# roymor1/OptimalStrategiesAgainstGenerativeAttacks

Measured on AMD Instinct MI355X. Metric: GIM episodes/sec (64x64x3, m=1 n=5 k=10), higher is better.
Workload: dtype f32

## Files before the change

### include/gim_hip.h

```cpp
#ifndef GIM_HIP_H
#define GIM_HIP_H

#include <stddef.h>
#include <stdint.h>

#ifdef __cplusplus
extern "C" {
#endif

#define GIM_OK 0
#define GIM_E_BADARG (-1)
#define GIM_E_LAUNCH (-2)

const char* gim_last_error(void);
int gim_version(void);

typedef struct {
    int32_t N, H, W, Cin, Cout, KH, ups;
    float pre_slope;
    int32_t pool, wfold, res_ups;
    int32_t tune_tile, tune_ksplit, tune_wgrad;
    int32_t out_zeroed;
    float post_slope;
    int32_t prec;
} gim_conv_shape;

int gim_conv2d_fold_weights(const float* w, float* f, int Cout, int Cin, int KH, void* stream);
typedef struct {
    const float* w;
    float* f;
    int32_t Cout, Cin, KH, reserved;
} gim_fold_job;
int gim_conv2d_fold_weights_batched(const gim_fold_job* jobs, const int32_t* tab, int n_blocks, void* stream);

int gim_conv2d_fwd(const float* x, const float* w, const float* bias, const float* sigma, const float* residual,
// ... 24 lines not shown
    int32_t Cout, Cin, KH, reserved;
} gim_sn_job;
int gim_spectral_sigma_batched(const gim_sn_job* jobs, int n_jobs, const int32_t* tab_cols, int n_col_blocks,
                               const int32_t* tab_rows, int n_row_blocks, float* out_base, int training, void* stream);

int gim_conv2d_transpose_weights(const float* w, float* wt, int Cout, int Cin, int KF, void* stream);
int gim_conv2d_dgrad_t(const float* dy, const float* wt, const float* sigma, const float* mask_x, float* dx,
                       const gim_conv_shape* shape, void* stream);

int gim_conv2d_xfold_weights(const float* w, float* wx, int Cout, int Cin, int KH, int J, void* stream);
int gim_conv2d_dgrad_xfold(const float* dy, const float* wx, const float* sigma, const float* mask_x, float* dx,
                           const gim_conv_shape* shape, int J, void* stream);

int gim_pad_image(const float* x, float* xp, int N, int H, int W, int C, int pad, float slope, void* stream);
int gim_conv2d_pack_rows_weights(const float* w, float* wp, int Cout, int Cin, int KH, void* stream);
int gim_conv2d_fwd_rows(const float* xp, const float* wp, const float* bias, const float* sigma, const float* residual,
                        float* y, const gim_conv_shape* shape, void* stream);
int gim_conv2d_wgrad_rows_acc(const float* dy, const float* xp, float* acc, float* bias_acc, const gim_conv_shape* shape, void* stream);

int gim_conv2d_pack_subpixel_weights(const float* wf, float* wm, int Cout, int Cin, int KH, void* stream);
int gim_depth_to_space2(const float* y4, const float* bias, float* y, int N, int Hs, int Ws, int C, float post_slope, void* stream);

int gim_conv_launch_plan(const gim_conv_shape* shape, int kind, int32_t* out);

int gim_conv2d_wgrad_acc(const float* dy, const float* x, float* acc, float* bias_acc, const gim_conv_shape* shape, void* stream);

typedef struct {
    const float* src;
    const float* bias_src;
    const float* w;
    const float* sigma;
    const float* u;
    const float* v;
    float* tmp;
    float* partial;
    float* grad_w;
    float* grad_b;
    int32_t Cout, Cin, K, fold;
    int32_t n_chunks, exclusive;
} gim_wgrad_job;
int gim_wgrad_finish_batched(const gim_wgrad_job* jobs, int n_jobs, const int32_t* tab, int n_blocks, const int32_t* tab_sn,
                             int n_blocks_sn, void* stream);

int gim_colsum(const float* x, float* out, float* scratch, int64_t rows, int C, void* stream);

int gim_colsum_acc(const float* x, float* out, float* scratch, int64_t rows, int C, void* stream);
// ... 154 lines not shown
```

### optimalstrategiesagainstgenerativeattacks_amd/_lib.py

```python
import ctypes
import os
from ctypes import POINTER, c_float, c_int, c_int32, c_int64, c_uint64, c_void_p

_HERE = os.path.dirname(os.path.abspath(__file__))
LIB_PATH = os.environ.get("GIM_LIB_PATH") or os.path.join(_HERE, "csrc", "libgim_hip.so")


class GimConvShape(ctypes.Structure):
    _fields_ = [("N", c_int32), ("H", c_int32), ("W", c_int32), ("Cin", c_int32), ("Cout", c_int32),
                ("KH", c_int32), ("ups", c_int32), ("pre_slope", c_float),
                ("pool", c_int32), ("wfold", c_int32), ("res_ups", c_int32),
                ("tune_tile", c_int32), ("tune_ksplit", c_int32), ("tune_wgrad", c_int32),
                ("out_zeroed", c_int32), ("post_slope", c_float), ("prec", c_int32)]


class GimInferConv(ctypes.Structure):
    _fields_ = [("N", c_int32), ("H", c_int32), ("W", c_int32), ("Cin", c_int32), ("Cout", c_int32),
                ("KH", c_int32), ("stride", c_int32)]


P = c_void_p
SP = POINTER(GimConvShape)


class GimFoldJob(ctypes.Structure):
    _fields_ = [("w", P), ("f", P), ("Cout", c_int32), ("Cin", c_int32), ("KH", c_int32), ("reserved", c_int32)]


class GimSnJob(ctypes.Structure):
    _fields_ = [("w", P), ("u", P), ("v", P), ("off_sigma", c_int64), ("off_u", c_int64), ("off_v", c_int64), ("off_scratch", c_int64),
                ("Cout", c_int32), ("Cin", c_int32), ("KH", c_int32), ("reserved", c_int32)]


class GimWgradJob(ctypes.Structure):
    _fields_ = [("src", P), ("bias_src", P), ("w", P), ("sigma", P), ("u", P), ("v", P), ("tmp", P), ("partial", P),
                ("grad_w", P), ("grad_b", P), ("Cout", c_int32), ("Cin", c_int32), ("K", c_int32), ("fold", c_int32),
# ... 35 lines not shown
    "gim_bgemm_grouped": [P, P, c_int, P],
    "gim_colsum_grouped": [P, P, c_int, P],
    "gim_scale_add_fwd": [P, P, P, P, c_int64, P],
    "gim_scale_add_fwd_act": [P, P, P, P, c_int64, c_float, P],
    "gim_scale_add_bwd": [P, P, P, P, P, P, c_int64, P],
    "gim_tanh_fwd": [P, P, c_int64, P],
    "gim_tanh_bwd": [P, P, P, c_int64, P],
    "gim_nchw_to_nhwc": [P, P, c_int, c_int, c_int, P],
    "gim_nhwc_to_nchw": [P, P, c_int, c_int, c_int, P],
    "gim_set_stats_fwd": [P, P, P, c_int, c_int, c_int, c_int64, c_int64, P],
    "gim_set_stats_bwd": [P, P, P, P, c_int, c_int, c_int, c_int64, c_int64, P],
    "gim_bce_logits_fwd": [P, P, c_float, c_int, P],
    "gim_bce_logits_bwd": [P, P, P, c_float, c_int, P],
    "gim_sum_dim1": [P, P, c_int, c_int, c_int, c_float, P],
    "gim_repeat_dim1": [P, P, c_int, c_int, c_int, c_float, P],
    "gim_noise_combine": [P, P, P, c_int, c_int, c_int, c_int, P],
    "gim_concat2": [P, P, P, c_int64, c_int, c_int, c_int, c_int, P],
    "gim_slice_channels": [P, P, c_int64, c_int, c_int, P],
    "gim_conv2d_wgrad_acc": [P, P, P, P, SP, P],
    "gim_wgrad_finish_batched": [P, c_int, P, c_int, P, c_int, P],
    "gim_colsum_acc": [P, P, P, c_int64, c_int, P],
    "gim_colsum2": [P, P, P, P, c_int, c_int, c_int, P],
    "gim_conv_launch_plan": [SP, c_int, P],
    "gim_conv2d_transpose_weights": [P, P, c_int, c_int, c_int, P],
    "gim_conv2d_dgrad_t": [P, P, P, P, P, SP, P],
    "gim_conv2d_xfold_weights": [P, P, c_int, c_int, c_int, c_int, P],
    "gim_conv2d_dgrad_xfold": [P, P, P, P, P, SP, c_int, P],
    "gim_episode_gather": [P, P, P, P, c_int, c_int, c_int, c_int, P],
    "gim_resize_bilinear_u8": [P, c_int64, c_int, c_int, c_int, c_int, P, c_int, c_int, P, P, c_int, P, P, c_int, P],
    "gim_maxpool_gather": [P, P, P, P, c_int, c_int, c_int, c_float, P],
    "gim_softmax_dim1_bwd_dp": [P, P, P, P, c_int, c_int, c_int, P],
    "gim_set_stats_bwd_bwd": [P, P, P, P, P, P, c_int, c_int, c_int, c_int64, c_int64, P],
    "gim_lrelu_mask_mul": [P, P, c_float, P, c_int64, P],
    "gim_sqsum_rows_fwd": [P, P, c_int, c_int64, P],
    "gim_sqsum_rows_bwd": [P, P, P, c_int, c_int64, P],
    "gim_img_att_mix_fwd": [P, P, P, P, P, P, P, P, c_int64, c_int, P],
    "gim_img_att_mix_bwd": [P, P, P, P, P, P, P, P, P, P, P, P, P, P, c_int64, c_int, P],
    "gim_adam_step": [P, P, P, P, c_int64, P, P, c_int, c_float, c_float, c_float, c_float, P, P],
    "gim_adam_step_scaled": [P, P, P, P, c_int64, P, P, c_int, c_float, c_float, c_float, c_float, P, P, P],
    "gim_spin": [c_int, P],
    "gim_pad_image": [P, P, c_int, c_int, c_int, c_int, c_int, c_float, P],
    "gim_conv2d_pack_rows_weights": [P, P, c_int, c_int, c_int, P],
    "gim_conv2d_pack_subpixel_weights": [P, P, c_int, c_int, c_int, P],
    "gim_depth_to_space2": [P, P, P, c_int, c_int, c_int, c_int, c_float, P],
    "gim_conv2d_fwd_rows": [P, P, P, P, P, P, SP, P],
    "gim_conv2d_wgrad_rows_acc": [P, P, P, P, SP, P],
# ... 61 lines not shown
```

### optimalstrategiesagainstgenerativeattacks_amd/csrc/conv_igemm.hip

```cpp
#include <stdlib.h>

#include "common.h"
#include <type_traits>

#define PM_MAX_PIXELS 16
#define PM_MIN_IMAGES 32
#define BK 16

struct Geo {
    int N, H, W, logH, logW;
    int Hin, Win;
    int ups;
    int s_in;
    int s_in_x;
    int off_y, off_x;
    int Th, Tw;
    int KF;
    int KFw;
    int wa_base, wa_step, wb_base, wb_step;
    int os, py, px;
    int pc, pc_kind, pc_K;
    int pm;
    unsigned long long pm_perm;
    unsigned long long pm_perm_cls[4];
// ... 856 lines not shown
    };
    epi_dispatch<EPI, BMODE>(p, has_res, has_mask, run);
}

struct WgP {
    Geo g;
    const float* dy;
    const float* x;
    float* slabs;
    float* bias_slabs;
    int Cin, Cout;
    int M;
    int Kcols;
    int mper;
    float pre_slope;
    float a_slope;
    const float* zero;
    unsigned x_bytes;
    float pos_inf;
    int atomic;
    int ns;
    int xcd;
    int pix;
};

__device__ __forceinline__ bool wgrad_block(const WgP& p, int& bx, int& by, int& bz) {
    if (!p.xcd) {
        bx = blockIdx.x; by = blockIdx.y; bz = blockIdx.z;
        return true;
    }
    const unsigned gx = gridDim.x, gy = gridDim.y;
    const unsigned L = blockIdx.x + gx * (blockIdx.y + gy * blockIdx.z);
    const unsigned xcd = L & 7u, q = L >> 3, ntiles = gx * gy;
    const unsigned tile = (q + xcd * ((ntiles + 7u) / 8u)) % ntiles, slice = (q / ntiles) * 8u + xcd;
    bx = (int)(tile % gx); by = (int)(tile / gx); bz = (int)slice;
    return slice < (unsigned)p.ns;
}

template <int BM, int BN, int TM, int TN, int VA, int VB, bool FASTB, int WBK = BK>
__global__ __launch_bounds__(256, 1) void conv_wgrad_kernel(const WgP p) {
    constexpr int WAVES_N = BN / (32 * TN);
    constexpr int WAVES_M = BM / (32 * TM);
    static_assert(WAVES_M * WAVES_N == 4, "4 waves per workgroup");
    static_assert(!FASTB || VB == 4, "fast B addressing: vector path only");
    constexpr int AU = BM / VA, BU = BN / VB;
    constexpr int A_RSTEP = 256 / AU, B_RSTEP = 256 / BU;
    constexpr int A_PER = (WBK + A_RSTEP - 1) / A_RSTEP, B_PER = (WBK + B_RSTEP - 1) / B_RSTEP;
    constexpr int A_FLOATS = WBK * BM, B_FLOATS = WBK * BN;
    __shared__ __attribute__((aligned(16))) float As[2][A_FLOATS];
    __shared__ __attribute__((aligned(16))) float Bs[2][B_FLOATS];

    const Geo& g = p.g;
    const int t = threadIdx.x;
    int bx, by, bz;
    if (!wgrad_block(p, bx, by, bz)) return;
    const int j0 = bx * BN, co0 = by * BM;
    const int mbeg = bz * p.mper;
    const int mend = min(p.M, mbeg + p.mper);
    const int He = g.Hin << g.ups, We = g.Win << g.ups;

    const int ac = (t % AU) * VA, ak = t / AU;
    const bool a_cok = (co0 + ac) < p.Cout;
    const int bc = (t % BU) * VB, bk = t / BU;
    const int j = j0 + bc;
    const bool b_jok = j < p.Kcols;
    const int tap = b_jok ? j / p.Cin : 0;
    const int ci = b_jok ? j - tap * p.Cin : 0;
    const int ta = tap / g.Tw, tb = tap - ta * g.Tw;
    const int dh = ta + g.off_y, dw = tb + g.off_x;
    const bool do_bias = p.bias_slabs != nullptr && bx == 0;

    constexpr bool fastb = FASTB;
    unsigned a_v[A_PER], b_l[B_PER];
    int b_dx[B_PER], b_dy[B_PER];
    const int b_bias = ((g.off_y < 0 ? -g.off_y : 0) * g.Win + (g.off_x < 0 ? -g.off_x : 0)) * p.pix * 4;
    const __amdgpu_buffer_rsrc_t rxb = __builtin_amdgcn_make_buffer_rsrc((void*)((const char*)p.x - b_bias), 0, p.x_bytes + (unsigned)b_bias, 0x00020000);
    if constexpr (VA == 4) {
#pragma unroll
        for (int i = 0; i < A_PER; ++i) {
            const int row = ak + i * A_RSTEP;
            a_v[i] = row < WBK ? (unsigned)((row * p.Cout + min(co0 + ac, p.Cout - 4)) * 4) : BUF_OOB;
        }
    }
    if constexpr (VB == 4) {
#pragma unroll
        for (int i = 0; i < B_PER; ++i) {
            const int row = bk + i * B_RSTEP;
            b_dy[i] = (row >> g.logW) * g.s_in + dh;
            b_dx[i] = (row & (g.W - 1)) * g.s_in + dw;
            b_l[i] = (b_jok && row < WBK) ? (unsigned)(((b_dy[i] * g.Win + b_dx[i]) * p.pix + ci) * 4 + b_bias) : BUF_OOB;
        }
    }

    float ra[A_PER][VA], rb[B_PER][VB];
    float bsum[VA];
#pragma unroll
    for (int e = 0; e < VA; ++e) bsum[e] = 0.f;

    auto load_tiles = [&](int mb) {
        if constexpr (VA == 4) {
            const int left = mend - mb;
            const __amdgpu_buffer_rsrc_t ra_rs = __builtin_amdgcn_make_buffer_rsrc(
                (void*)(p.dy + (long long)mb * p.Cout), 0, (unsigned)min(left, WBK) * (unsigned)p.Cout * 4u, 0x00020000);
#pragma unroll
            for (int i = 0; i < A_PER; ++i) {
                const f32x4 val = buf_load4(ra_rs, a_v[i], 0);
#pragma unroll
                for (int e = 0; e < 4; ++e) ra[i][e] = val[e];
            }
        } else {
#pragma unroll
            for (int i = 0; i < A_PER; ++i) {
                const int row = ak + i * A_RSTEP;
                const int m = mb + row;
                const bool v = a_cok && row < WBK && m < mend;
                ra[i][0] = v ? p.dy[(long long)m * p.Cout + co0 + ac] : 0.f;
            }
        }
        if constexpr (VB == 4) {
            if constexpr (fastb) {
                const int n = mb >> (g.logH + g.logW);
                const int oys = ((mb >> g.logW) & (g.H - 1)) * g.s_in, oxs = (mb & (g.W - 1)) * g.s_in;
// ... 70 lines not shown
#pragma unroll
        for (int i = 0; i < B_PER; ++i) {
            const int row = bk + i * B_RSTEP;
            if (row < WBK) {
                if constexpr (VB == 4) {
                    f32x4 val = {rb[i][0], rb[i][1], rb[i][2], rb[i][3]};
                    *reinterpret_cast<f32x4*>(&Bs[buf][row * BN + bc]) = val;
                } else {
                    Bs[buf][row * BN + bc] = rb[i][0];
                }
            }
        }
    };

    const int lane = t & 63, r = lane & 31, h = lane >> 5, wv = t >> 6;
    const int wm0 = (wv / WAVES_N) * 32 * TM, wn0 = (wv % WAVES_N) * 32 * TN;
    f32x16 acc[TM][TN];
#pragma unroll
    for (int i = 0; i < TM; ++i)
#pragma unroll
        for (int jj = 0; jj < TN; ++jj)
#pragma unroll
            for (int e = 0; e < 16; ++e) acc[i][jj][e] = 0.f;
    const int nk = (mend > mbeg) ? (mend - mbeg + WBK - 1) / WBK : 0;
    if (nk > 0) {
        load_tiles(mbeg);
        store_tiles(0);
    }
    __syncthreads();
    const float* a_rd = &As[0][0] + h * BM + wm0 + r;
    const float* b_rd = &Bs[0][0] + h * BN + wn0 + r;
    auto kstep32 = [&](int ks, auto BUFC, auto MAINC) {
        constexpr int buf = decltype(BUFC)::value;
        constexpr bool MAIN = decltype(MAINC)::value;
        if (MAIN || ks + 1 < nk) load_tiles(mbeg + (ks + 1) * WBK);
        __builtin_amdgcn_sched_barrier(0);
#pragma unroll
        for (int kp = 0; kp < WBK / 2; ++kp) {
            float a[TM], b[TN];
#pragma unroll
            for (int i = 0; i < TM; ++i) a[i] = a_rd[buf * A_FLOATS + 2 * kp * BM + 32 * i];
#pragma unroll
            for (int jj = 0; jj < TN; ++jj) b[jj] = b_rd[buf * B_FLOATS + 2 * kp * BN + 32 * jj];
#pragma unroll
            for (int i = 0; i < TM; ++i)
#pragma unroll
                for (int jj = 0; jj < TN; ++jj)
// ... 905 lines not shown
    g.os = 1;
    return g;
}

extern "C" int gim_conv2d_fwd_rows(const float* xp, const float* wp, const float* bias, const float* sigma, const float* residual,
                                   float* y, const gim_conv_shape* s, void* stream) {
    int rc = rows_shape_ok(s);
    if (rc) return rc;
    GIM_CHECK_ARG(xp && wp && y && !((uintptr_t)xp & 15) && !((uintptr_t)wp & 15), "conv fwd (rows form): null or unaligned pointer");
    ConvCall c{};
    ConvP& p = c.p;
    const int CaP = (s->KH * s->Cin + 15) & ~15;
    rc = convp_begin(p, geo_rows(s), CaP, s->Cout, s->Cin, 6, s, "conv fwd (rows form): the padded image batch exceeds 2 GiB (32-bit buffer offsets): split the batch");
    if (rc) return rc;
    p.x = xp; p.w = wp; p.bias = bias; p.sigma = sigma; p.res = residual; p.mask_x = nullptr; p.y = y;
    p.Cin_w = CaP;
    p.pre_slope = 1.f; p.mask_slope = 1.f; p.out_scale = 1.f; p.res_ups = 0;
    GIM_CHECK_ARG(s->post_slope >= 0.f && s->post_slope <= 1.f, "conv fwd: post_slope must be in [0, 1] (0 or 1 = none)");
    p.post_slope = (s->post_slope > 0.f) ? s->post_slope : 1.f;
    c.y_elems = (size_t)s->N * s->H * s->W * s->Cout;
    GIM_CHECK_ARG(c.y_elems * sizeof(float) <= 0x7FFFFFF0ull, "conv: the output exceeds 2 GiB (32-bit buffer offsets): split the batch");
    return plan_and_run(c, stream, "gim_conv2d_fwd_rows");
}
template <int VA, int VB, bool FASTB>
static void launch_wgrad(const WgP& p, int bm, int bn, int bk, dim3 g, hipStream_t st) {
    if constexpr (VA == 4 && VB == 4) {
        if (bk == 32 && bm == 64 && bn == 64) {
            hipLaunchKernelGGL((conv_wgrad_kernel<64, 64, 1, 1, 4, 4, FASTB, 32>), g, dim3(256), 0, st, p);
            return;
        }
    }
    if (bm == 128 && bn == 128) hipLaunchKernelGGL((conv_wgrad_kernel<128, 128, 2, 2, VA, VB, FASTB>), g, dim3(256), 0, st, p);
    else if (bm == 128 && bn == 64) hipLaunchKernelGGL((conv_wgrad_kernel<128, 64, 2, 1, VA, VB, FASTB>), g, dim3(256), 0, st, p);
    else if (bm == 64 && bn == 128) hipLaunchKernelGGL((conv_wgrad_kernel<64, 128, 1, 2, VA, VB, FASTB>), g, dim3(256), 0, st, p);
    else if (bm == 64 && bn == 64) hipLaunchKernelGGL((conv_wgrad_kernel<64, 64, 1, 1, VA, VB, FASTB>), g, dim3(256), 0, st, p);
    else hipLaunchKernelGGL((conv_wgrad_kernel<32, 128, 1, 1, VA, VB, FASTB>), g, dim3(256), 0, st, p);
}

constexpr int NARROW_PARTS = 16, NARROW_MPER = 512, NARROW_U = 8, NARROW_ROWS = NARROW_MPER / NARROW_PARTS;
template <int CN, bool EXACT>
__global__ __launch_bounds__(64 * NARROW_PARTS) void wgrad_1x1_narrow_kernel(const float* __restrict__ wide, const float* __restrict__ nar,
                                                                             float* __restrict__ out, float* __restrict__ bias_out, int M, int Cw,
                                                                             int Cn_, float slope_x, int wide_is_dy) {
    __shared__ float red[NARROW_PARTS][9][64];
    const int Cn = EXACT ? CN : Cn_;
    const int lane = threadIdx.x & 63, part = __builtin_amdgcn_readfirstlane(threadIdx.x >> 6);
    const int c = blockIdx.y * 64 + lane, cc = min(c, Cw - 1);
    const int m0 = blockIdx.x * NARROW_MPER, m1 = min(M, m0 + NARROW_MPER);
    float acc[CN], bsum = 0.f;
#pragma unroll
    for (int j = 0; j < CN; ++j) acc[j] = 0.f;
    const int mw = m0 + part * NARROW_ROWS, me = min(m1, mw + NARROW_ROWS);
    for (int mb = mw; mb < me; mb += NARROW_U) {
        float wv[NARROW_U], nv[NARROW_U][CN];
        const float* nrow = nar + (long long)mb * Cn;
#pragma unroll
        for (int u = 0; u < NARROW_U; ++u) {
            wv[u] = wide[(long long)(mb + u) * Cw + cc];
#pragma unroll
// ... 46 lines not shown
            float v = 0.f;
            for (int q = 0; q < 64; ++q) v += red[0][threadIdx.x][q];
            atomicAdd(&bias_out[threadIdx.x], v);
        }
    }
}

enum WgFamily { WG_MFMA = 0, WG_MFMA_F16, WG_TINY, WG_ROW, WG_NARROW };
enum WgCombine { WG_SLABS = 0, WG_ONE_SLAB, WG_ACC };
struct WgPlan {
    int family;
    int rows, cols, M;
    int ns;
    int atomic;
    int bm, bn, bk, xcd;
    int slices, mper;
    int gx, gy, gz;
    int table_hit;
};

static WgPlan wgrad_plan(const gim_conv_shape* s0, bool rows_form, int combine, bool aligned) {
    WgPlan q{};
    gim_conv_shape v = *s0;
    if (rows_form) {
        v.tune_tile = s0->tune_tile ? s0->tune_tile : -1;
        v.prec = 0;
    }
    const gim_conv_shape* s = &v;
    const bool up_fold = s->ups && s->wfold;
    const int KF = s->wfold ? s->KH + 1 : s->KH;
    q.rows = up_fold ? s->Cin : s->Cout;
    q.cols = KF * KF * (up_fold ? s->Cout : s->Cin);
    const long long M = (long long)s->N * (s->H >> (s->wfold ? 1 : 0)) * (s->W >> (s->wfold ? 1 : 0));
    q.M = (int)M;
    int target = s->tune_wgrad > 0 ? s->tune_wgrad : 0;
    int tile = s->tune_tile > 0 ? s->tune_tile : 0;
    if (!target && !tile && s->tune_tile == 0) {
        const int pcw = (s->pool ? 1 : 0) + (up_fold ? 2 : 0);
        const TuneEntry* te = tune_lookup(2, (int)M, q.rows, q.cols, s->KH, pcw);
        if (te) { target = te->ks; tile = te->tile; q.table_hit = 1; }
    }
    bool row_resident = false;
    int row_target = 0;
    if (tile >= 20000) { row_resident = true; row_target = target; tile -= 20000; }
    const bool f16 = s->prec >= 1 && q.rows % 4 == 0 && (up_fold ? s->Cout : s->Cin) % 4 == 0 && q.rows >= 32 && q.cols >= 64;
    if (f16) { row_resident = false; tile = 128; if (!(s->tune_wgrad > 0)) target = 0; q.table_hit = 0; }
// ... 75 lines not shown
    if (rc) return rc;
    GIM_CHECK_ARG(dy && x && slabs, "conv wgrad: null pointer");
    q = wgrad_plan(s, rows, prezeroed ? WG_ACC : (n_slabs == 1 ? WG_ONE_SLAB : WG_SLABS), !((uintptr_t)dy & 15) && !((uintptr_t)x & 15));
    if (!prezeroed) GIM_CHECK_ARG(n_slabs == 1 || n_slabs == q.ns, "conv wgrad: n_slabs must be 1 (atomic combine) or gim_conv2d_wgrad_slabs(shape)");
    const bool up_fold = s->ups && s->wfold;
    GIM_CHECK_ARG(!(up_fold && bias_slabs), "conv wgrad: the sub-pixel form does not produce the bias gradient (use gim_colsum)");
    p = WgP{};
    p.zero = zero_page();
    p.pos_inf = __builtin_inff();
    if (rows) p.g = geo_rows(s);
    else if (s->pool || up_fold) p.g = geo_s2(s, false);
    else p.g = geo_plain(s, false);
    if (up_fold) {
        p.dy = x; p.x = dy; p.Cin = s->Cout; p.Cout = s->Cin; p.pre_slope = 1.f; p.a_slope = s->pre_slope; p.pix = s->Cout;
    } else {
        p.dy = dy; p.x = x; p.Cin = s->Cin; p.Cout = s->Cout; p.pre_slope = s->pre_slope; p.a_slope = 1.f; p.pix = s->Cin;
    }
    p.slabs = slabs; p.bias_slabs = bias_slabs;
    p.M = q.M; p.Kcols = q.cols; p.mper = q.mper; p.ns = q.slices; p.xcd = q.xcd; p.atomic = q.atomic;
    if (rows) { p.Cin = (s->KH * s->Cin + 15) & ~15; p.pix = s->Cin; p.pre_slope = 1.f; }
    const unsigned long long xb = (unsigned long long)p.g.N * p.g.Hin * p.g.Win * p.pix * 4ull;
    GIM_CHECK_ARG(xb <= 0x7FFFFFF0ull, "conv wgrad: gathered tensor larger than 2 GiB (32-bit buffer offsets): split the batch");
    p.x_bytes = (unsigned)xb;
    return GIM_OK;
}

static int wgrad_impl(const float* dy, const float* x, float* slabs, float* bias_slabs, int n_slabs, const gim_conv_shape* s,
                      void* stream, bool prezeroed, bool rows = false) {
    WgP p;
    WgPlan q;
    const int rc = wgrad_call(p, q, dy, x, slabs, bias_slabs, n_slabs, s, prezeroed, rows);
    if (rc) return rc;
    hipStream_t st = (hipStream_t)stream;
    if (!prezeroed && (q.atomic || q.family == WG_TINY)) {
        (void)hipMemsetAsync(slabs, 0, (size_t)q.rows * q.cols * sizeof(float), st);
        if (bias_slabs) (void)hipMemsetAsync(bias_slabs, 0, (size_t)q.rows * sizeof(float), st);
    }
    const dim3 g(q.gx, q.gy, q.gz);
    switch (q.family) {
    case WG_TINY:
        gim_tiny_wgrad_acc(dy, x, slabs, bias_slabs, s, st);
        break;
    case WG_ROW:
        if (s->W >= 16) hipLaunchKernelGGL(conv_wgrad_row_kernel<16>, g, dim3(256), 0, st, p);
        else if (s->W == 8) hipLaunchKernelGGL(conv_wgrad_row_kernel<8>, g, dim3(256), 0, st, p);
        else hipLaunchKernelGGL(conv_wgrad_row_kernel<4>, g, dim3(256), 0, st, p);
        break;
    case WG_NARROW: {
        const int wide_is_dy = s->Cin <= 8 ? 1 : 0;
        const int Cw = wide_is_dy ? s->Cout : s->Cin, Cn = wide_is_dy ? s->Cin : s->Cout;
        const dim3 b(64 * NARROW_PARTS);
        const float *wd = wide_is_dy ? dy : x, *nr = wide_is_dy ? x : dy;
        if (Cn == 3) hipLaunchKernelGGL((wgrad_1x1_narrow_kernel<3, true>), g, b, 0, st, wd, nr, slabs, bias_slabs, q.M, Cw, Cn, s->pre_slope, wide_is_dy);
        else if (Cn == 6) hipLaunchKernelGGL((wgrad_1x1_narrow_kernel<6, true>), g, b, 0, st, wd, nr, slabs, bias_slabs, q.M, Cw, Cn, s->pre_slope, wide_is_dy);
        else hipLaunchKernelGGL((wgrad_1x1_narrow_kernel<8, false>), g, b, 0, st, wd, nr, slabs, bias_slabs, q.M, Cw, Cn, s->pre_slope, wide_is_dy);
        break;
    }
    default: {
        const bool va = (p.Cout % 4 == 0) && !((uintptr_t)p.dy & 15);
        const bool vb = (p.Cin % 4 == 0) && !((uintptr_t)p.x & 15);
        const int bk = (q.bk == 32 && va && vb) ? 32 : BK;
        const bool fastb = vb && p.g.ups == 0 && ((p.g.H * p.g.W) & (bk - 1)) == 0;
        const bool f16 = q.family == WG_MFMA_F16 && va && vb && bk == 32, sat = s->prec != 2;
        if (f16 && fastb) hipLaunchKernelGGL((sat ? conv_wgrad_f16_kernel<true, true> : conv_wgrad_f16_kernel<true, false>), g, dim3(256), 0, st, p);
        else if (f16) hipLaunchKernelGGL((sat ? conv_wgrad_f16_kernel<false, true> : conv_wgrad_f16_kernel<false, false>), g, dim3(256), 0, st, p);
        else if (va && fastb) launch_wgrad<4, 4, true>(p, q.bm, q.bn, bk, g, st);
        else if (va && vb) launch_wgrad<4, 4, false>(p, q.bm, q.bn, bk, g, st);
        else if (va) launch_wgrad<4, 1, false>(p, q.bm, q.bn, bk, g, st);
        else if (vb) launch_wgrad<1, 4, false>(p, q.bm, q.bn, bk, g, st);
        else launch_wgrad<1, 1, false>(p, q.bm, q.bn, bk, g, st);
    }
    }
    return gim_check_launch("gim_conv2d_wgrad");
}

extern "C" int gim_conv2d_wgrad(const float* dy, const float* x, float* slabs, float* bias_slabs, int n_slabs,
                                const gim_conv_shape* s, void* stream) {
    return wgrad_impl(dy, x, slabs, bias_slabs, n_slabs, s, stream, false);
}

extern "C" int gim_conv2d_wgrad_acc(const float* dy, const float* x, float* acc, float* bias_acc, const gim_conv_shape* s, void* stream) {
    int rc = check_shape(s);
    if (rc) return rc;
    size_t xi, yi;
    image_elems(s, false, xi, yi);
    gim_conv_shape a, b;
    if (split_batch(*s, xi > yi ? xi : yi, a, b)) {
        rc = gim_conv2d_wgrad_acc(dy, x, acc, bias_acc, &a, stream);
// ... 30 lines not shown
    if (split_batch(*s, xi > yi ? xi : yi, a, b)) {
        rc = launch_plan(&a, kind, out);
        return rc ? rc : launch_plan(&b, kind, out);
    }
    if (kind == 3) {
        const int form[] = {0, 2, 3, 1, 0};
        WgP p;
        WgPlan q;
        rc = wgrad_call(p, q, fake, fake, fake, nullptr, 1, s, true, false);
        if (!rc) plan_row(out, q.table_hit, q.bm, q.bn, q.slices, q.gx, q.gy, q.gz, form[q.family]);
        return rc;
    }
    const int form[] = {0, 1, 2, 2};
    ConvCall c;
    rc = kind == 0 ? fwd_call(c, fake, fake, nullptr, nullptr, nullptr, fake, s)
                   : dgrad_call(c, fake, fake, nullptr, nullptr, fake, s, kind == 2, nullptr, 0.f);
    if (rc) return rc;
    const IgemmPlan q = plan_igemm(c.p, c.bmode, c.gen);
    const int skipped = 1000 - pm_valid_permille(c.p.g, c.p.M, q.BM);
    plan_row(out, q.table_hit, q.BM, q.BN, q.ksplit, q.gx, q.gy, q.gz, form[q.family] | (skipped << 8));
    return GIM_OK;
}

extern "C" int gim_conv_launch_plan(const gim_conv_shape* s, int kind, int32_t* out) {
    GIM_CHECK_ARG(s && out && kind >= 0 && kind <= 3, "conv_launch_plan: bad args");
    for (int i = 0; i < 8; ++i) out[i] = -1;
    return launch_plan(s, kind, out);
}
```

### optimalstrategiesagainstgenerativeattacks_amd/ops.py

```python
import collections
import ctypes
import math
import os
import struct
import warnings
import weakref

import torch
from torch.autograd import Function
from torch.autograd.function import once_differentiable

from . import _lib, optim
from ._lib import GimConvShape, GimGemmJob, GimWgradJob, check

LRELU_SLOPE = 0.2

_HIGHER = {"input_grad_only": False}


class input_grad_only:
    def __enter__(self):
        self.prev = _HIGHER["input_grad_only"]
        _HIGHER["input_grad_only"] = True

# ... 185 lines not shown
    def __init__(self, scaler):
        self.on = 1 if scaler is not None else 0

    def __enter__(self):
        _ARMED[0] += self.on

    def __exit__(self, *exc):
        _ARMED[0] -= self.on


def set_matrix_path(name):
    if name not in ("fp32", "fp16"):
        raise ValueError("matrix path must be 'fp32' or 'fp16'")
    prev = matrix_path()
    _PREC[0] = 1 if name == "fp16" else 0
    if prev != name:
        _SPLITS_K.clear()
    return prev


_SHAPES = {}


def _shape(N, H, W, Cin, Cout, KH, ups, pre_slope, pool=0, wfold=0, res_ups=0):
    prec = 2 if (_PREC[0] and _ARMED[0]) else _PREC[0]
    key = (N, H, W, Cin, Cout, KH, ups, pre_slope, pool, wfold, res_ups, _DETERMINISTIC[0], prec)
    t = _SHAPES.get(key)
    if t is None:
        t = _SHAPES[key] = GimConvShape(N, H, W, Cin, Cout, KH, ups, pre_slope, pool, wfold, res_ups, 0, 1 if _DETERMINISTIC[0] else 0, 0, 0, 0.0,
                                        prec if H * W > 1 else 0)
    return GimConvShape.from_buffer_copy(t)


_TUNE_OVERRIDE = {}


def _tuned(sh, kind, key):
    ov = _TUNE_OVERRIDE.get((kind, key)) if _TUNE_OVERRIDE else None
    if ov is not None:
        sh.tune_tile = ov[0]
        if kind == "wgrad":
            sh.tune_wgrad = ov[1]
        else:
            sh.tune_ksplit = ov[1]
    return sh


_ZERO_POOL = os.environ.get("GIM_NO_ZERO_POOL") is None
_SPLITS_K = {}
_ZERO_PAGES = {}
_ZERO_PAGE = 16 << 20
_Plan = collections.namedtuple("_Plan", "ksplit skipped_permille")


def _launch_plan(sh, plan_kind, key):
    k_ = (plan_kind,) + key
    v = _SPLITS_K.get(k_)
    if v is None:
        out = (ctypes.c_int32 * 8)()
        check(_lib.load().gim_conv_launch_plan(ctypes.byref(sh), plan_kind, ctypes.cast(out, ctypes.c_void_p)), "conv_launch_plan")
        v = _SPLITS_K[k_] = _Plan(out[3], out[7] >> 8)
    return v


def _zeros_from_pool(shape, device):
    n = 1
    for d in shape:
        n *= d
    na = (n + 63) & ~63
    if na > _ZERO_PAGE >> 1:
        return torch.zeros(shape, device=device, dtype=torch.float32)
    raw = (torch._C._cuda_getDevice(), _stream())
    pg = _ZERO_PAGES.get(raw)
    if pg is None or pg[1] + na > pg[0].numel():
        pg = _ZERO_PAGES[raw] = [torch.zeros(_ZERO_PAGE, device=device, dtype=torch.float32), 0]
    v = pg[0][pg[1]:pg[1] + n].view(shape)
    pg[1] += na
    return v


def _conv_out(sh, plan_kind, key, shape, device):
    if _ZERO_POOL and _launch_plan(sh, plan_kind, key).ksplit > 1 and not torch.cuda.is_current_stream_capturing():
        sh.out_zeroed = 1
        return _zeros_from_pool(shape, device)
# ... 471 lines not shown
    elif route == "t":
        wt = _transposed(lib, w, wk, Cout, Cin, KH + 1 if g.fold else KH)
        dx = _conv_out(sh, 2, g.key, tuple(x.shape), x.device)
        check(lib.gim_conv2d_dgrad_t(_p(dy), _p(wt), _p(sigma), _p(mask), _p(dx), sh, st), "conv2d_dgrad_t")
    elif route == "ups":
        dxu = _conv_out(sh, 1, g.key, (N, H, W, Cin), dy.device)
        dx = torch.empty_like(x)
        check(lib.gim_conv2d_dgrad(_p(dy), _p(wk), _p(sigma), None, _p(dxu), sh, st), "conv2d_dgrad")
        check(lib.gim_upsample2x_bwd(_p(dxu), _p(mask), g.pre_slope, _p(dx), N, H >> 1, W >> 1, Cin, st), "upsample2x_bwd")
    else:
        dx = _conv_out(sh, 1, g.key, tuple(x.shape), x.device)
        if route == "res":
            check(lib.gim_conv2d_dgrad_res(_p(dy), _p(wk), _p(sigma), _p(mask), _p(_req(res_half, "res_half")), 0.25, _p(dx), sh, st), "conv2d_dgrad_res")
        else:
            check(lib.gim_conv2d_dgrad(_p(dy), _p(wk), _p(sigma), _p(mask), _p(dx), sh, st), "conv2d_dgrad")
    if add_res:
        out = torch.empty_like(dx)
        check(lib.gim_add_avgpool2_bwd(_p(dx), _p(_req(res_half, "res_half")), _p(out), N, H, W, Cin, st), "add_avgpool2_bwd")
        return out
    return dx


def _conv_wgrad(lib, dy, x, w, wp, bias, sigma, u_s, v_s, sh, g, want_b, st, xp=None):
    if _FLOPS is not None:
        _note_conv("wgrad", g)
    Cin, Cout, KH, ups, fold = g.Cin, g.Cout, g.KH, g.ups, g.fold
    dev = dy.device
    dw = db = None
    Mo, K, KFF = g.out_pixels, g.K, g.KFF
    slab_bias = want_b and not (fold and ups)
    acc_w = _grad_target(w) if (sigma is not None or not fold) and not torch.is_grad_enabled() else None
    acc_b = _grad_target(bias) if (slab_bias and acc_w is not None) else None
    route, ns = _wgrad_route(g, sh, acc_w is not None, sigma is not None, want_b and slab_bias and acc_b is None,
                             xp is not None and dy.is_contiguous())
    fold_code = (2 if ups else 1) if fold else 0
    queued = route in ("queued", "queued_rows")
    if queued:
        q = _queue()
        n = Cout * K
        if Cout * KFF >= 1 << 31:
            raise RuntimeError("weight gradient of more than 2^31 elements (gim_wgrad_finish_batched indexes with 32 bits)")
        n_chunks = (n + q.CHUNK - 1) // q.CHUNK
        rows = route == "queued_rows"
        src = q.take(Cout * KH * ((KH * Cin + 15) & ~15) if rows else Cout * KFF, dev)
        bsrc = q.take(Cout, dev) if slab_bias else None
        sn = sigma is not None
        tmp = q.take(n, dev) if ((fold or rows) and sn) else None
        part = q.take(n_chunks, dev) if sn else None
        if rows:
            check(lib.gim_conv2d_wgrad_rows_acc(_p(dy), _p(xp), src, bsrc, sh, st), "conv2d_wgrad_rows_acc")
        else:
            check(lib.gim_conv2d_wgrad_acc(_p(dy), _p(x), src, bsrc, sh, st), "conv2d_wgrad_acc")
        q.add((src, bsrc or 0, _p(wp) if sn else 0, _p(sigma) or 0, _p(u_s) or 0, _p(v_s) or 0, tmp or 0, part or 0,
               _p(acc_w), _p(acc_b) or 0, Cout, Cin, KH, 3 if rows else fold_code, n_chunks), (sigma, u_s, v_s))
    else:
        dwp = torch.empty(Cout * K, device=dev, dtype=torch.float32)
        if want_b and acc_b is None:
            db = torch.empty(Cout, device=dev, dtype=torch.float32)
        if route == "direct":
# ... 1543 lines not shown
```

Measured before the change: 436.3.

## Add position-major wgrad kernel that skips padded-out pixel positions on small images

Adds a position-major variant of the MFMA weight-gradient kernel for small spatial sizes (at most 16 pixels, batch a multiple of 16). It walks pixels grouped by output position across images and uses a per-column-block bitmask to skip positions where the kernel tap falls entirely in padding, cutting wasted MACs on tiny feature maps. An env flag can force the old image-major order, and a helper reports the skipped fraction for FLOP accounting. This adds more complex indexing and a new dy buffer resource, and changes the accumulation order.

```diff
diff --git a/include/gim_hip.h b/include/gim_hip.h
--- a/include/gim_hip.h
+++ b/include/gim_hip.h
@@ -11,6 +11,7 @@
 #define GIM_OK 0
 #define GIM_E_BADARG (-1)
 #define GIM_E_LAUNCH (-2)
+#define GIM_WGRAD_IMAGE_MAJOR 0x40000000
 
 const char* gim_last_error(void);
 int gim_version(void);
@@ -81,6 +82,8 @@
 int gim_depth_to_space2(const float* y4, const float* bias, float* y, int N, int Hs, int Ws, int C, float post_slope, void* stream);
 
 int gim_conv_launch_plan(const gim_conv_shape* shape, int kind, int32_t* out);
+
+int gim_conv_wgrad_skipped(const gim_conv_shape* shape, int32_t* permille);
 
 int gim_conv2d_wgrad_acc(const float* dy, const float* x, float* acc, float* bias_acc, const gim_conv_shape* shape, void* stream);
 
diff --git a/optimalstrategiesagainstgenerativeattacks_amd/_lib.py b/optimalstrategiesagainstgenerativeattacks_amd/_lib.py
--- a/optimalstrategiesagainstgenerativeattacks_amd/_lib.py
+++ b/optimalstrategiesagainstgenerativeattacks_amd/_lib.py
@@ -12,6 +12,9 @@
                 ("pool", c_int32), ("wfold", c_int32), ("res_ups", c_int32),
                 ("tune_tile", c_int32), ("tune_ksplit", c_int32), ("tune_wgrad", c_int32),
                 ("out_zeroed", c_int32), ("post_slope", c_float), ("prec", c_int32)]
+
+
+WGRAD_IMAGE_MAJOR = 0x40000000
 
 
 class GimInferConv(ctypes.Structure):
@@ -93,6 +96,7 @@
     "gim_colsum_acc": [P, P, P, c_int64, c_int, P],
     "gim_colsum2": [P, P, P, P, c_int, c_int, c_int, P],
     "gim_conv_launch_plan": [SP, c_int, P],
+    "gim_conv_wgrad_skipped": [SP, P],
     "gim_conv2d_transpose_weights": [P, P, c_int, c_int, c_int, P],
     "gim_conv2d_dgrad_t": [P, P, P, P, P, SP, P],
     "gim_conv2d_xfold_weights": [P, P, c_int, c_int, c_int, c_int, P],
diff --git a/optimalstrategiesagainstgenerativeattacks_amd/csrc/conv_igemm.hip b/optimalstrategiesagainstgenerativeattacks_amd/csrc/conv_igemm.hip
--- a/optimalstrategiesagainstgenerativeattacks_amd/csrc/conv_igemm.hip
+++ b/optimalstrategiesagainstgenerativeattacks_amd/csrc/conv_igemm.hip
@@ -902,7 +902,22 @@
     int ns;
     int xcd;
     int pix;
+    unsigned dy_bytes;
 };
+
+__host__ __device__ __forceinline__ unsigned long long wgrad_pm_positions(const Geo& g, int Cin, int Kcols, int j0, int bn) {
+    const int jend = j0 + bn < Kcols ? j0 + bn : Kcols;
+    unsigned long long mask = 0;
+    for (int tap = j0 / Cin; tap <= (jend - 1) / Cin; ++tap) {
+        const int ta = tap / g.Tw, tb = tap - ta * g.Tw;
+        unsigned long long cols = 0;
+        for (int ox = 0; ox < g.W; ++ox)
+            if ((unsigned)(ox * g.s_in + tb + g.off_x) < (unsigned)g.Win) cols |= 1ull << ox;
+        for (int oy = 0; oy < g.H; ++oy)
+            if ((unsigned)(oy * g.s_in + ta + g.off_y) < (unsigned)g.Hin) mask |= cols << (oy * g.W);
+    }
+    return mask;
+}
 
 __device__ __forceinline__ bool wgrad_block(const WgP& p, int& bx, int& by, int& bz) {
     if (!p.xcd) {
@@ -917,12 +932,14 @@
     return slice < (unsigned)p.ns;
 }
 
-template <int BM, int BN, int TM, int TN, int VA, int VB, bool FASTB, int WBK = BK>
+template <int BM, int BN, int TM, int TN, int VA, int VB, bool FASTB, int WBK = BK, bool PMAJ = false>
 __global__ __launch_bounds__(256, 1) void conv_wgrad_kernel(const WgP p) {
     constexpr int WAVES_N = BN / (32 * TN);
     constexpr int WAVES_M = BM / (32 * TM);
     static_assert(WAVES_M * WAVES_N == 4, "4 waves per workgroup");
     static_assert(!FASTB || VB == 4, "fast B addressing: vector path only");
+    static_assert(!PMAJ || (VA == 4 && VB == 4 && !FASTB && WBK % 16 == 0), "position-major pixels: vector path only");
+    constexpr int NU = WBK / 16;
     constexpr int AU = BM / VA, BU = BN / VB;
     constexpr int A_RSTEP = 256 / AU, B_RSTEP = 256 / BU;
     constexpr int A_PER = (WBK + A_RSTEP - 1) / A_RSTEP, B_PER = (WBK + B_RSTEP - 1) / B_RSTEP;
@@ -955,14 +972,27 @@
     int b_dx[B_PER], b_dy[B_PER];
     const int b_bias = ((g.off_y < 0 ? -g.off_y : 0) * g.Win + (g.off_x < 0 ? -g.off_x : 0)) * p.pix * 4;
     const __amdgpu_buffer_rsrc_t rxb = __builtin_amdgcn_make_buffer_rsrc((void*)((const char*)p.x - b_bias), 0, p.x_bytes + (unsigned)b_bias, 0x00020000);
-    if constexpr (VA == 4) {
+    if constexpr (PMAJ) {
+#pragma unroll
+        for (int i = 0; i < A_PER; ++i) {
+            const int row = ak + i * A_RSTEP;
+            a_v[i] = row < WBK ? (unsigned)(((row & 15) * g.H * g.W * p.Cout + min(co0 + ac, p.Cout - 4)) * 4) : BUF_OOB;
+        }
+#pragma unroll
+        for (int i = 0; i < B_PER; ++i) {
+            const int row = bk + i * B_RSTEP;
+            b_dy[i] = dh; b_dx[i] = dw;
+            b_l[i] = (b_jok && row < WBK) ? (unsigned)((((row & 15) * g.Hin * g.Win + dh * g.Win + dw) * p.pix + ci) * 4 + b_bias) : BUF_OOB;
+        }
+    }
+    if constexpr (!PMAJ && VA == 4) {
 #pragma unroll
         for (int i = 0; i < A_PER; ++i) {
             const int row = ak + i * A_RSTEP;
             a_v[i] = row < WBK ? (unsigned)((row * p.Cout + min(co0 + ac, p.Cout - 4)) * 4) : BUF_OOB;
         }
     }
-    if constexpr (VB == 4) {
+    if constexpr (!PMAJ && VB == 4) {
 #pragma unroll
         for (int i = 0; i < B_PER; ++i) {
             const int row = bk + i * B_RSTEP;
@@ -971,6 +1001,33 @@
             b_l[i] = (b_jok && row < WBK) ? (unsigned)(((b_dy[i] * g.Win + b_dx[i]) * p.pix + ci) * 4 + b_bias) : BUF_OOB;
         }
     }
+    int u_pos = 0, u_n = 0, pm_units = 0;
+    unsigned long long u_rem = 0;
+    [[maybe_unused]] const __amdgpu_buffer_rsrc_t rdy = __builtin_amdgcn_make_buffer_rsrc((void*)p.dy, 0, p.dy_bytes, 0x00020000);
+    if constexpr (PMAJ) {
+        const int P = g.H * g.W;
+        const unsigned long long all = P < 64 ? (1ull << P) - 1ull : ~0ull;
+        const unsigned long long valid = do_bias ? all : wgrad_pm_positions(g, p.Cin, p.Kcols, j0, BN);
+        u_pos = mbeg / g.N;
+        u_n = mbeg - u_pos * g.N;
+        u_rem = valid >> u_pos;
+        for (int pos = u_pos; pos < P && pos * g.N < mend; ++pos)
+            if ((valid >> pos) & 1ull) pm_units += (min(mend, (pos + 1) * g.N) - max(mbeg, pos * g.N)) >> 4;
+        if (pm_units == 0 && p.atomic) return;
+    }
+    auto next_unit = [&](int& pos, int& n) -> bool {
+        const int sk = u_rem ? __builtin_ctzll(u_rem) : 64;
+        u_n = sk ? 0 : u_n;
+        u_pos += sk;
+        u_rem = sk < 64 ? u_rem >> sk : 0ull;
+        pos = u_pos; n = u_n;
+        const bool ok = u_pos * g.N + u_n < mend;
+        const int wrap = (u_n + 16 >= g.N) ? 1 : 0;
+        u_n = wrap ? 0 : u_n + 16;
+        u_pos += wrap;
+        u_rem >>= wrap;
+        return ok;
+    };
 
     float ra[A_PER][VA], rb[B_PER][VB];
     float bsum[VA];
@@ -978,6 +1035,34 @@
     for (int e = 0; e < VA; ++e) bsum[e] = 0.f;
 
     auto load_tiles = [&](int mb) {
+        if constexpr (PMAJ) {
+            unsigned sa[NU], sb[NU];
+            bool uok[NU], bv[NU];
+#pragma unroll
+            for (int u = 0; u < NU; ++u) {
+                int pos, n;
+                uok[u] = next_unit(pos, n);
+                const int oys = (pos >> g.logW) * g.s_in, oxs = (pos & (g.W - 1)) * g.s_in;
+                sa[u] = (unsigned)((n * g.H * g.W + pos) * p.Cout) * 4u;
+                sb[u] = (unsigned)(((n * g.Hin + oys) * g.Win + oxs) * p.pix) * 4u;
+                bv[u] = uok[u] && (unsigned)(oys + b_dy[0]) < (unsigned)He && (unsigned)(oxs + b_dx[0]) < (unsigned)We;
+            }
+#pragma unroll
+            for (int i = 0; i < A_PER; ++i) {
+                const int u = (i * A_RSTEP) / 16;
+                const f32x4 val = buf_load4(rdy, uok[u] ? a_v[i] : BUF_OOB, sa[u]);
+#pragma unroll
+                for (int e = 0; e < 4; ++e) ra[i][e] = val[e];
+            }
+#pragma unroll
+            for (int i = 0; i < B_PER; ++i) {
+                const int u = (i * B_RSTEP) / 16;
+                const f32x4 val = buf_load4(rxb, bv[u] ? b_l[i] : BUF_OOB, sb[u]);
+#pragma unroll
+                for (int e = 0; e < 4; ++e) rb[i][e] = val[e];
+            }
+            return;
+        }
         if constexpr (VA == 4) {
             const int left = mend - mb;
             const __amdgpu_buffer_rsrc_t ra_rs = __builtin_amdgcn_make_buffer_rsrc(
@@ -1094,7 +1179,7 @@
         for (int jj = 0; jj < TN; ++jj)
 #pragma unroll
             for (int e = 0; e < 16; ++e) acc[i][jj][e] = 0.f;
-    const int nk = (mend > mbeg) ? (mend - mbeg + WBK - 1) / WBK : 0;
+    const int nk = PMAJ ? (pm_units + NU - 1) / NU : ((mend > mbeg) ? (mend - mbeg + WBK - 1) / WBK : 0);
     if (nk > 0) {
         load_tiles(mbeg);
         store_tiles(0);
@@ -2046,19 +2131,19 @@
     GIM_CHECK_ARG(c.y_elems * sizeof(float) <= 0x7FFFFFF0ull, "conv: the output exceeds 2 GiB (32-bit buffer offsets): split the batch");
     return plan_and_run(c, stream, "gim_conv2d_fwd_rows");
 }
-template <int VA, int VB, bool FASTB>
+template <int VA, int VB, bool FASTB, bool PMAJ = false>
 static void launch_wgrad(const WgP& p, int bm, int bn, int bk, dim3 g, hipStream_t st) {
     if constexpr (VA == 4 && VB == 4) {
         if (bk == 32 && bm == 64 && bn == 64) {
-            hipLaunchKernelGGL((conv_wgrad_kernel<64, 64, 1, 1, 4, 4, FASTB, 32>), g, dim3(256), 0, st, p);
+            hipLaunchKernelGGL((conv_wgrad_kernel<64, 64, 1, 1, 4, 4, FASTB, 32, PMAJ>), g, dim3(256), 0, st, p);
             return;
         }
     }
-    if (bm == 128 && bn == 128) hipLaunchKernelGGL((conv_wgrad_kernel<128, 128, 2, 2, VA, VB, FASTB>), g, dim3(256), 0, st, p);
-    else if (bm == 128 && bn == 64) hipLaunchKernelGGL((conv_wgrad_kernel<128, 64, 2, 1, VA, VB, FASTB>), g, dim3(256), 0, st, p);
-    else if (bm == 64 && bn == 128) hipLaunchKernelGGL((conv_wgrad_kernel<64, 128, 1, 2, VA, VB, FASTB>), g, dim3(256), 0, st, p);
-    else if (bm == 64 && bn == 64) hipLaunchKernelGGL((conv_wgrad_kernel<64, 64, 1, 1, VA, VB, FASTB>), g, dim3(256), 0, st, p);
-    else hipLaunchKernelGGL((conv_wgrad_kernel<32, 128, 1, 1, VA, VB, FASTB>), g, dim3(256), 0, st, p);
+    if (bm == 128 && bn == 128) hipLaunchKernelGGL((conv_wgrad_kernel<128, 128, 2, 2, VA, VB, FASTB, BK, PMAJ>), g, dim3(256), 0, st, p);
+    else if (bm == 128 && bn == 64) hipLaunchKernelGGL((conv_wgrad_kernel<128, 64, 2, 1, VA, VB, FASTB, BK, PMAJ>), g, dim3(256), 0, st, p);
+    else if (bm == 64 && bn == 128) hipLaunchKernelGGL((conv_wgrad_kernel<64, 128, 1, 2, VA, VB, FASTB, BK, PMAJ>), g, dim3(256), 0, st, p);
+    else if (bm == 64 && bn == 64) hipLaunchKernelGGL((conv_wgrad_kernel<64, 64, 1, 1, VA, VB, FASTB, BK, PMAJ>), g, dim3(256), 0, st, p);
+    else hipLaunchKernelGGL((conv_wgrad_kernel<32, 128, 1, 1, VA, VB, FASTB, BK, PMAJ>), g, dim3(256), 0, st, p);
 }
 
 constexpr int NARROW_PARTS = 16, NARROW_MPER = 512, NARROW_U = 8, NARROW_ROWS = NARROW_MPER / NARROW_PARTS;
@@ -2151,6 +2236,7 @@
 static WgPlan wgrad_plan(const gim_conv_shape* s0, bool rows_form, int combine, bool aligned) {
     WgPlan q{};
     gim_conv_shape v = *s0;
+    v.tune_wgrad &= ~GIM_WGRAD_IMAGE_MAJOR;
     if (rows_form) {
         v.tune_tile = s0->tune_tile ? s0->tune_tile : -1;
         v.prec = 0;
@@ -2272,7 +2358,39 @@
     const unsigned long long xb = (unsigned long long)p.g.N * p.g.Hin * p.g.Win * p.pix * 4ull;
     GIM_CHECK_ARG(xb <= 0x7FFFFFF0ull, "conv wgrad: gathered tensor larger than 2 GiB (32-bit buffer offsets): split the batch");
     p.x_bytes = (unsigned)xb;
+    const unsigned long long db = (unsigned long long)q.M * p.Cout * 4ull;
+    p.dy_bytes = db <= 0x7FFFFFF0ull ? (unsigned)db : 0x7FFFFFF0u;
     return GIM_OK;
+}
+
+#ifndef WG_PM_MAX_PIXELS
+#define WG_PM_MAX_PIXELS 16
+#endif
+static_assert(WG_PM_MAX_PIXELS <= 64, "position-major pixels: the position mask is 64 bits");
+struct WgVec { bool va, vb, fastb, pm; int bk; };
+static WgVec wgrad_vec(const WgP& p, const WgPlan& q, const gim_conv_shape* s, bool rows) {
+    WgVec v{};
+    v.va = (p.Cout % 4 == 0) && !((uintptr_t)p.dy & 15);
+    v.vb = (p.Cin % 4 == 0) && !((uintptr_t)p.x & 15);
+    v.bk = (q.bk == 32 && v.va && v.vb) ? 32 : BK;
+    v.fastb = v.vb && p.g.ups == 0 && ((p.g.H * p.g.W) & (v.bk - 1)) == 0;
+    const Geo& g = p.g;
+    const int P = g.H * g.W;
+    v.pm = q.family == WG_MFMA && v.va && v.vb && !rows && g.ups == 0 && g.s_in == 1 && !s->wfold && p.pix == p.Cin && g.Th * g.Tw > 1 &&
+           P <= WG_PM_MAX_PIXELS && g.N % 16 == 0 && g.N >= v.bk && q.mper % 16 == 0 &&
+           (unsigned long long)q.M * p.Cout * 4ull <= 0x7FFFFFF0ull && !(s->tune_wgrad & GIM_WGRAD_IMAGE_MAJOR);
+    if (v.pm) v.fastb = false;
+    return v;
+}
+
+static int wgrad_pm_skipped_permille(const WgP& p, const WgPlan& q) {
+    const int P = p.g.H * p.g.W;
+    long long skipped = 0, total = 0;
+    for (int bx = 0; bx < q.gx; ++bx) {
+        skipped += P - __builtin_popcountll(wgrad_pm_positions(p.g, p.Cin, p.Kcols, bx * q.bn, q.bn));
+        total += P;
+    }
+    return (int)((skipped * 1000 + total / 2) / total);
 }
 
 static int wgrad_impl(const float* dy, const float* x, float* slabs, float* bias_slabs, int n_slabs, const gim_conv_shape* s,
@@ -2307,13 +2425,13 @@
         break;
     }
     default: {
-        const bool va = (p.Cout % 4 == 0) && !((uintptr_t)p.dy & 15);
-        const bool vb = (p.Cin % 4 == 0) && !((uintptr_t)p.x & 15);
-        const int bk = (q.bk == 32 && va && vb) ? 32 : BK;
-        const bool fastb = vb && p.g.ups == 0 && ((p.g.H * p.g.W) & (bk - 1)) == 0;
+        const WgVec v = wgrad_vec(p, q, s, rows);
+        const bool va = v.va, vb = v.vb, fastb = v.fastb;
+        const int bk = v.bk;
         const bool f16 = q.family == WG_MFMA_F16 && va && vb && bk == 32, sat = s->prec != 2;
         if (f16 && fastb) hipLaunchKernelGGL((sat ? conv_wgrad_f16_kernel<true, true> : conv_wgrad_f16_kernel<true, false>), g, dim3(256), 0, st, p);
         else if (f16) hipLaunchKernelGGL((sat ? conv_wgrad_f16_kernel<false, true> : conv_wgrad_f16_kernel<false, false>), g, dim3(256), 0, st, p);
+        else if (v.pm) launch_wgrad<4, 4, false, true>(p, q.bm, q.bn, bk, g, st);
         else if (va && fastb) launch_wgrad<4, 4, true>(p, q.bm, q.bn, bk, g, st);
         else if (va && vb) launch_wgrad<4, 4, false>(p, q.bm, q.bn, bk, g, st);
         else if (va) launch_wgrad<4, 1, false>(p, q.bm, q.bn, bk, g, st);
@@ -2390,6 +2508,27 @@
     return GIM_OK;
 }
 
+extern "C" int gim_conv_wgrad_skipped(const gim_conv_shape* s, int32_t* permille) {
+    GIM_CHECK_ARG(s && permille, "conv_wgrad_skipped: bad args");
+    *permille = 0;
+    float* const fake = reinterpret_cast<float*>(uintptr_t(4096));
+    int rc = check_shape(s);
+    if (rc) return rc;
+    size_t xi, yi;
+    image_elems(s, false, xi, yi);
+    gim_conv_shape a, b;
+    if (split_batch(*s, xi > yi ? xi : yi, a, b)) {
+        rc = gim_conv_wgrad_skipped(&a, permille);
+        return rc ? rc : gim_conv_wgrad_skipped(&b, permille);
+    }
+    WgP p;
+    WgPlan q;
+    rc = wgrad_call(p, q, fake, fake, fake, nullptr, 1, s, true, false);
+    if (rc) return rc;
+    if (q.family == WG_MFMA && wgrad_vec(p, q, s, false).pm) *permille = wgrad_pm_skipped_permille(p, q);
+    return GIM_OK;
+}
+
 extern "C" int gim_conv_launch_plan(const gim_conv_shape* s, int kind, int32_t* out) {
     GIM_CHECK_ARG(s && out && kind >= 0 && kind <= 3, "conv_launch_plan: bad args");
     for (int i = 0; i < 8; ++i) out[i] = -1;
diff --git a/optimalstrategiesagainstgenerativeattacks_amd/ops.py b/optimalstrategiesagainstgenerativeattacks_amd/ops.py
--- a/optimalstrategiesagainstgenerativeattacks_amd/ops.py
+++ b/optimalstrategiesagainstgenerativeattacks_amd/ops.py
@@ -231,12 +231,15 @@
 _SHAPES = {}
 
 
+_WGRAD_FLAGS = _lib.WGRAD_IMAGE_MAJOR if os.environ.get("GIM_WGRAD_IMAGE_MAJOR") is not None else 0
+
+
 def _shape(N, H, W, Cin, Cout, KH, ups, pre_slope, pool=0, wfold=0, res_ups=0):
     prec = 2 if (_PREC[0] and _ARMED[0]) else _PREC[0]
     key = (N, H, W, Cin, Cout, KH, ups, pre_slope, pool, wfold, res_ups, _DETERMINISTIC[0], prec)
     t = _SHAPES.get(key)
     if t is None:
-        t = _SHAPES[key] = GimConvShape(N, H, W, Cin, Cout, KH, ups, pre_slope, pool, wfold, res_ups, 0, 1 if _DETERMINISTIC[0] else 0, 0, 0, 0.0,
+        t = _SHAPES[key] = GimConvShape(N, H, W, Cin, Cout, KH, ups, pre_slope, pool, wfold, res_ups, 0, 1 if _DETERMINISTIC[0] else 0, _WGRAD_FLAGS, 0, 0.0,
                                         prec if H * W > 1 else 0)
     return GimConvShape.from_buffer_copy(t)
 
@@ -249,7 +252,7 @@
     if ov is not None:
         sh.tune_tile = ov[0]
         if kind == "wgrad":
-            sh.tune_wgrad = ov[1]
+            sh.tune_wgrad = ov[1] | _WGRAD_FLAGS
         else:
             sh.tune_ksplit = ov[1]
     return sh
@@ -268,7 +271,12 @@
     if v is None:
         out = (ctypes.c_int32 * 8)()
         check(_lib.load().gim_conv_launch_plan(ctypes.byref(sh), plan_kind, ctypes.cast(out, ctypes.c_void_p)), "conv_launch_plan")
-        v = _SPLITS_K[k_] = _Plan(out[3], out[7] >> 8)
+        skipped = out[7] >> 8
+        if plan_kind == 3:
+            pm = ctypes.c_int32(0)
+            check(_lib.load().gim_conv_wgrad_skipped(ctypes.byref(sh), ctypes.cast(ctypes.byref(pm), ctypes.c_void_p)), "conv_wgrad_skipped")
+            skipped = pm.value
+        v = _SPLITS_K[k_] = _Plan(out[3], skipped)
     return v
 
 
@@ -786,8 +794,6 @@
 
 
 def _conv_wgrad(lib, dy, x, w, wp, bias, sigma, u_s, v_s, sh, g, want_b, st, xp=None):
-    if _FLOPS is not None:
-        _note_conv("wgrad", g)
     Cin, Cout, KH, ups, fold = g.Cin, g.Cout, g.KH, g.ups, g.fold
     dev = dy.device
     dw = db = None
@@ -799,6 +805,8 @@
                              xp is not None and dy.is_contiguous())
     fold_code = (2 if ups else 1) if fold else 0
     queued = route in ("queued", "queued_rows")
+    if _FLOPS is not None:
+        _note_conv("wgrad", g, *((sh, 3) if route != "queued_rows" else ()))
     if queued:
         q = _queue()
         n = Cout * K
```

Result: no change. 434.5 (-0.4%).
